# GlassyWing/yolo_deepsort

Measured on AMD Instinct MI355X. Metric: end-to-end frames/sec (detect+ReID+assoc), 608x608, higher is better.
Workload: dtype f16x3

## Files before the change

include/ydsort.h:

```cpp
#ifndef YDSORT_H
#define YDSORT_H

#include <stddef.h>
#include <stdint.h>

#ifdef __cplusplus
extern "C" {
#endif

typedef struct yds_net yds_net;
typedef struct yds_reid yds_reid;
typedef struct yds_trk yds_trk;
typedef struct yds_pipe yds_pipe;
typedef struct yds_zones yds_zones;
typedef struct yds_heatmap yds_heatmap;
typedef struct yds_act yds_act;
typedef struct yds_ident yds_ident;
typedef struct yds_comm yds_comm;

int yds_init(int device_id);
int yds_current_device(void);
int yds_device_pci_bus_id(char *buf, int len);
const char *yds_last_error(void);
int yds_device_count(void);
// ... 13 lines not shown
int yds_darknet_set_batch_max(yds_net *, int batch_max);
int yds_darknet_batch_max(const yds_net *);
int yds_darknet_set_half(yds_net *, int on);
int yds_darknet_layer_format(const yds_net *, int layer);
int yds_darknet_num_boxes(const yds_net *);
int yds_darknet_num_attrs(const yds_net *);
int yds_darknet_num_layers(const yds_net *);
int yds_darknet_layer_shape(const yds_net *, int layer, int *c, int *h, int *w);
int64_t yds_darknet_conv_flops(const yds_net *);
int yds_darknet_forward_f32(yds_net *, const float *nchw_host, int batch, float *out_host);
int yds_darknet_forward_u8(yds_net *, const uint8_t *rgb_hwc_host, int h, int w, int batch,
                           float *out_host_or_null);
int yds_darknet_forward_u8_dev(yds_net *, const uint8_t *rgb_hwc_dev, int h, int w, int batch);
int yds_darknet_forward_u8_mixed_dev(yds_net *, const uint8_t *rgb_hwc_dev, const uint64_t *frame_off, const int32_t *frame_hw ,
                                     size_t frames_bytes, int batch);
const uint8_t *yds_darknet_last_frames_dev(yds_net *, int *h, int *w, int *batch);
int yds_darknet_layer_output(yds_net *, int layer, int batch, float *nchw_host);
int yds_darknet_get_input(yds_net *, int batch, float *nchw_host);

int yds_nms(yds_net *, int image, float conf_thres, double iou_thres, int frame_h, int frame_w,
            float *out6_host, int cap, int *n_out);
int yds_nms_pred(const float *pred_host, int n_boxes, int attrs, float conf_thres, double iou_thres,
                 float *out6_host, int cap, int *n_out);

int yds_detect_tiled(yds_net *, const uint8_t *rgb_hwc_host, int h, int w, const int32_t *tiles_xyhw, int n_tiles,
                     float conf_thres, double iou_thres, float *out6_host, int cap, int *n_out);
int yds_nms_merge_pred(const float *pred_host, int n_boxes, int attrs, float conf_thres, double iou_thres,
                       float *out6_host, int cap, int *n_out);
int yds_nms_merge_pred_batched(const float *pred_host, int n_frames, int n_boxes, int attrs, float conf_thres, double iou_thres,
                               float *out6_host, int cap, int *n_out);
int yds_nms_ragged_pred(const float *pred_host, size_t total_rows, int attrs, int n_frames, const uint64_t *row0, const int32_t *n_rows,
                        const int32_t *corner_merge, const float *scale, float conf_thres, double iou_thres, float *out6_host, int cap,
                        int *n_out);

yds_reid *yds_reid_create(int max_crops);
void yds_reid_destroy(yds_reid *);
int yds_reid_load_tensor(yds_reid *, const char *name, const float *data_host, const int64_t *shape, int ndim);
int yds_reid_finalize(yds_reid *);
int64_t yds_reid_flops_per_crop(void);
int yds_reid_embed(yds_reid *, const uint8_t *frame_rgb_host, int h, int w, const float *tlwh_host,
                   int D, float *out_host);
int yds_reid_embed_dev(yds_reid *, const uint8_t *frame_rgb_dev, int h, int w, const float *tlwh_host,
                       int D, float *out_host_or_null);
const float *yds_reid_features_dev(yds_reid *);
int yds_reid_preprocess(yds_reid *, const uint8_t *frame_rgb_host, int h, int w, const float *tlwh_host,
                        int D, float *nchw_host);
// ... 240 lines not shown
```

yolo_deepsort_amd/_lib.py:

```python

from __future__ import annotations

import ctypes as C
import os

import numpy as np

HERE = os.path.dirname(os.path.abspath(__file__))
_TAG = os.environ.get("YDS_BUILD_TAG", "")
LIB_PATH = os.path.join(HERE, "libydsort" + ("_" + _TAG if _TAG else "") + ".so")


class YdsError(RuntimeError):
    pass


_P = C.c_void_p
_I = C.c_int
_F = C.c_float
_D = C.c_double
_SZ = C.c_size_t
_I64 = C.c_int64

SIGNATURES = {
# ... 170 lines not shown
    "yds_pipeline_set_zones": (_I, [_P, _P]),
    "yds_pipeline_last_zone_events": (_I, [_P, _P, _P, _I, _P]),
    "yds_heatmap_create": (_P, [_I, _I]),
    "yds_heatmap_destroy": (None, [_P]),
    "yds_heatmap_set_stream": (_I, [_P, _I, _I, _I, _I, _I]),
    "yds_heatmap_reset": (_I, [_P, _I]),
    "yds_heatmap_update": (_I, [_P, _P, _P, _P, _P, _I, _P]),
    "yds_heatmap_get_layers": (_I, [_P, _I, _P, _SZ]),
    "yds_heatmap_get_max": (_I, [_P, _I, _I, _P]),
    "yds_heatmap_get_tracks": (_I, [_P, _I, _P, _P, _P, _P, _P, _I, _P]),
    "yds_heatmap_render": (_I, [_P, _P, _I, _P, _P, _I, _I, _I, _I, _I64, _I, _P]),
    "yds_heatmap_set_timing": (_I, [_P, _I]),
    "yds_heatmap_last_us": (_I, [_P, _I, _P]),
    "yds_pipeline_set_heatmap": (_I, [_P, _P]),
    "yds_overlay_tracks_masked": (_I, [_P, _I, _P, _I, _I, _I, _P, _P, _P, _I, _P, _P, _I, _I, _I, _P, _P, _I, _I, C.c_uint32, _P, _P]),
    "yds_overlay_tracks_bgr_masked": (_I, [_P, _I, _P, _I, _I, _I, _P, _P, _P, _I, _P, _P, _I, _I, _I, _P, _P, _I, _I, C.c_uint32, _P]),
    "yds_anonymize_frames": (_I, [_P, _I, _P, _I, _I, _I, _P, _P, _I, _I, C.c_uint32]),
    "yds_pipeline_last_detections": (_I, [_P, _P, _I, _P]),
    "yds_overlay_tracks_mixed": (_I, [_P, _SZ, _I, _P, _P, _P, _I, _P, _P, _P, _I, _P, _P, _I, _I, _P, _P, _I, _I, C.c_uint32, _P, _SZ, _P]),
    "yds_overlay_tracks_bgr_mixed": (_I, [_P, _SZ, _I, _P, _P, _P, _I, _P, _P, _P, _I, _P, _P, _I, _I, _P, _P, _I, _I, C.c_uint32, _P]),
    "yds_anonymize_frames_mixed": (_I, [_P, _SZ, _I, _P, _P, _P, _I, _P, _P, _I, _I, C.c_uint32]),
    "yds_overlay_set_timing": (_I, [_I]),
    "yds_overlay_last_us": (_I, [_P]),
}

_lib = None
MISSING = []


def load():
    global _lib
    if _lib is not None:
        return _lib
    if not os.path.exists(LIB_PATH):
        raise YdsError(f"{LIB_PATH} not found: build it with `python -m yolo_deepsort_amd.build` "
                       "(the product has no CPU fallback)")
    lib = C.CDLL(LIB_PATH)
    for name, (res, args) in SIGNATURES.items():
        try:
            fn = getattr(lib, name)
        except AttributeError:
            MISSING.append(name)
            continue
        fn.restype = res
        fn.argtypes = args
    _lib = lib
# ... 128 lines not shown
```

yolo_deepsort_amd/csrc/common.h:

```cpp
#pragma once
#include <hip/hip_runtime.h>
#include <stdint.h>
#include <stdio.h>
#include <string>
#include <vector>
#include <stdexcept>

#include "slot_plan.h"

namespace yds {

void set_error(const std::string &msg);
struct Error : std::runtime_error {
    explicit Error(const std::string &m) : std::runtime_error(m) {}
};
[[noreturn]] void fail(const char *fmt, ...);
int bound_device();
void bind_thread();
hipStream_t make_stream(bool latency_role);

#define YDS_HIP(expr)                                                                          \
    do {                                                                                       \
        hipError_t _e = (expr);                                                                \
        if (_e != hipSuccess)                                                                  \
// ... 86 lines not shown
int launch_conv(const ConvArgs &a, hipStream_t s, int variant = -1);
constexpr int kVariantMask = 0xff, kTileGnShift = 8;
bool conv_presplit_input(const ConvArgs &a);
bool launch_conv_maxpool3s2(const ConvArgs &a, hipStream_t s);
int conv_autotune(const ConvArgs &a, hipStream_t s, float *best_us);
std::vector<int> conv_candidates(const ConvArgs &a);
enum ConvMath { MATH_F32 = 0, MATH_F16X3 = 1 };
int conv_math();
void set_conv_math(int m);
void pack_weights_f16x3(const float *w, int cout, int kpad, std::vector<uint16_t> &out);
const char *conv_variant_name(int v);
double conv_flops(const ConvArgs &a);
double conv_bytes_io(const View &v);
double conv_bytes(const ConvArgs &a);

void launch_maxpool(const View &x, const View &y, int k, int stride, int pad, bool zero_pad_br, hipStream_t s);
void launch_upsample(const View &x, const View &y, int stride, hipStream_t s);
void launch_copy(const View &x, const View &y, hipStream_t s);
void launch_add(const View &a, const View &b, const View &y, hipStream_t s);
void launch_nchw_to_nhwc(const float *src_nchw, const View &y, int c_src, hipStream_t s);
void launch_nhwc_to_nchw(const View &x, float *dst_nchw, hipStream_t s);
void nhwc_to_host(const View &x, float *dst_nchw_host, hipStream_t s);
void launch_pack_h16(const float *src_f32, const View &y, hipStream_t s);
void launch_yolo_decode(const View &head, float *out, int total_boxes, int box_off, int num_classes,
                        const float *anchors_wh , int A, int img_h, int img_w, hipStream_t s);
void launch_inject(const View &head, int image, const float *rows_dev, int n, int head_index, int num_classes,
                   float logit, hipStream_t s);
void launch_inject_batch(const View &head, int batch, const float *table_dev, const int *offsets_dev, int max_rows, int head_index,
                         int num_classes, float logit, hipStream_t s);
void launch_resize_u8(const uint8_t *frames, int n, int h, int w, const View &y, hipStream_t s, bool bgr = false);
std::vector<FrameGeom> checked_layout(const uint64_t *frame_off, const int32_t *frame_hw, int n, size_t frames_bytes);
void launch_slot_resize(const uint8_t *frames, const SlotRec *slots, int n, const View &y, hipStream_t s, bool bgr);
void launch_slot_boxes(const float *pred, int n_boxes, int attrs, const SlotRec *slots, int n, float *dst, hipStream_t s);
struct ReidFront {
    const uint8_t *frames = nullptr;
    const FrameGeom *geom = nullptr;
    const int *boxes = nullptr;
    int h = 0, w = 0, bgr = 0;
};
void launch_crop_resize(const ReidFront &f, int D, const View &y, hipStream_t s);
void launch_reid_stem(const ReidFront &f, int D, const float *w, int kpad, const float *bias, const View &pooled, hipStream_t s);
constexpr int kReidStemUnitsPerCrop = 4;
int reid_stem_grid();
void launch_avgpool_l2norm(const View &x, float *out, hipStream_t s);

}
```

yolo_deepsort_amd/csrc/darknet.cpp:

```cpp
#include "engine.h"
#include "h16.h"
#include "conv_common.h"

#include <math.h>
#include <stdlib.h>
#include <string.h>
#include <map>
#include <sstream>

namespace yds {

std::vector<CfgBlock> parse_cfg(const std::string &text) {
    std::vector<CfgBlock> blocks;
    std::istringstream in(text);
    std::string line;
    auto strip = [](std::string s) {
        size_t a = s.find_first_not_of(" \t\r\n"), b = s.find_last_not_of(" \t\r\n");
        return a == std::string::npos ? std::string() : s.substr(a, b - a + 1);
    };
    while (std::getline(in, line)) {
        if (line.empty() || line[0] == '#') continue;
        line = strip(line);
        if (line.empty()) fail("cfg: whitespace-only line (the reference parser rejects it too)");
        if (line[0] == '[') {
// ... 584 lines not shown
        switch (st.kind) {
        case Step::CONV: case Step::CONV_MERGED: case Step::CONV_STEM2: case Step::CONV_BLOCK1:
            enqueue_conv(st, first, batch, stream);
            break;
        case Step::MAXPOOL: launch_maxpool(v(st.src), v(i), st.ksize, st.stride, st.pad, st.zero_br, stream); break;
        case Step::UPSAMPLE: launch_upsample(v(l.src), v(i), l.stride, stream); break;
        case Step::COPY: {
            View d = v(i);
            d.p += fmt_slots(d.fmt, st.arg);
            launch_copy(v(st.src), d, stream);
            break;
        }
        case Step::ADD: launch_add(v(l.refs[0]), v(l.refs[1]), v(i), stream); break;
        case Step::YOLO: {
            const View head = v(l.src);
            const int hidx = st.arg;
            if (inject_active && inject_set >= 0) {
                launch_inject_batch(head, batch, inject_table.p, inject_offsets_dev.p + (size_t)inject_set * batch_max + first, inject_max_rows, hidx,
                                    l.classes, inject_logit, stream);
            } else {
                for (int b = 0; b < batch && inject_active; ++b)
                    launch_inject(head, b, inject_rows[first + b].p, inject_n[first + b], hidx, l.classes, inject_logit, stream);
            }
            launch_yolo_decode(head, out.p + (size_t)first * total_boxes * attrs, total_boxes, l.box_off, l.classes, l.anchors.data(), (int)l.anchors.size() / 2, img_h, img_w, stream);
            break;
        }
        }
    }
}

void Darknet::forward_f32_host(const float *nchw, int batch, float *out_host) {
    size_t n = (size_t)batch * in_channels * img_h * img_w;
    YDS_HIP(hipMemcpyAsync(stage_f32.p, nchw, n * sizeof(float), hipMemcpyHostToDevice, stream));
    launch_nchw_to_nhwc(stage_f32.p, input_view(batch), in_channels, stream);
    run_graph(batch);
    if (out_host) YDS_HIP(hipMemcpyAsync(out_host, out.p, (size_t)batch * total_boxes * attrs * sizeof(float), hipMemcpyDeviceToHost, stream));
    YDS_HIP(hipStreamSynchronize(stream));
}

void Darknet::forward_u8_dev(const uint8_t *frames_dev, int h, int w, int batch) {
    if (in_channels != 3) fail("forward_u8: network expects %d channels", in_channels);
    check_pass(batch);
    launch_resize_u8(frames_dev, batch, h, w, input_view(batch), stream);
    run_graph(batch);
}

void Darknet::forward_u8_frames_dev(const uint8_t *frames_dev, const std::vector<FrameGeom> &geom) {
// ... 283 lines not shown
```

yolo_deepsort_amd/csrc/engine.h:

```cpp
#pragma once
#include "common.h"
#include "conv_weights.h"

#include <map>
#include <memory>
#include <string>
#include <utility>
#include <vector>

namespace yds {

struct CfgBlock {
    std::string type;
    std::map<std::string, std::string> kv;
};
std::vector<CfgBlock> parse_cfg(const std::string &text);

enum LayerType { L_CONV, L_MAXPOOL, L_UPSAMPLE, L_ROUTE, L_SHORTCUT, L_YOLO };

struct Layer {
    LayerType type = L_CONV;
    int c = 0, h = 0, w = 0;
    int root = -1, coff = 0;
    int src = -1;
// ... 70 lines not shown
    bool half_mode = false;
    void set_half(bool on);
    void plan_half_formats();
    int owner_of(int layer, int &off) const;
    int total_boxes = 0, attrs = 0;
    std::vector<Layer> layers;
    std::vector<Storage> storage;
    std::vector<int> yolo_layers;
    DevBuf<float> input, out, stage_f32;
    DevBuf<uint8_t> stage_u8;
    DevBuf<SlotRec> slot_tab;
    int stage_h = 0, stage_w = 0, stage_n = 0;
    DevBuf<float> tiled_pred;
    hipStream_t stream = nullptr;
    std::vector<DevBuf<float>> inject_rows;
    std::vector<int> inject_n;
    bool inject_active = false;
    DevBuf<float> inject_table;
    std::vector<int> inject_offsets;
    DevBuf<int> inject_offsets_dev;
    int inject_max_rows = 0;
    int inject_set = -1;
    float inject_logit = 6.f;
    struct ConvTimeRec { hipEvent_t e0 = nullptr, e1 = nullptr; int variant = 0; double flops = 0, bytes = 0, attain_us = 0; };
    bool time_convs = false;
    std::vector<ConvTimeRec> conv_pending;
    std::vector<hipEvent_t> ev_pool;
    hipEvent_t timing_event();
    void resolve_conv_timing();
    double conv_us[kConvVariants] = {}, conv_flops_acc[kConvVariants] = {}, conv_bytes_acc[kConvVariants] = {}, conv_attain_us[kConvVariants] = {};
    int64_t conv_launches[kConvVariants] = {};

private:
    void allocate_buffers();
    void check_pass(int batch) const;
    void run_graph(int batch);
    void run_lane(int first, int batch, hipStream_t st, int l0 = 0, int l1 = -1);
    void enqueue_conv(const Step &st, int first, int batch, hipStream_t s);
    const LaunchPlan &plan(int batch);
    LaunchPlan plan_;
    int plan_epoch = 0;
    bool stem_fusable = false;
    int block1_at = -1;
    std::vector<hipStream_t> lane_streams;
    std::vector<hipEvent_t> lane_done;
    hipEvent_t lane_fork = nullptr;
};

struct NmsUniform { int32_t n_boxes, corner, merge; float sx, sy; };
class NmsWorkspace {
public:
    explicit NmsWorkspace(int max_candidates = 16384, int frames = 1);
    ~NmsWorkspace();
    NmsWorkspace(const NmsWorkspace &) = delete;
    void launch(const float *pred_dev, const NmsUniform &u, int n_frames, int attrs, float conf_thres, double iou_thres, int cap, hipStream_t s);
    void launch(const float *pred_dev, const NmsFrame *fr, int n_frames, int max_rows, size_t total_rows, int attrs, float conf_thres,
                double iou_thres, int cap, hipStream_t s);
    int collect(int frame, float *out6_host, int cap);
    void resize(int max_candidates, int n_frames);
    int needed(int n_frames) const;
    static constexpr int kMaxCandidates = 1 << 18;
    int run(const float *pred_dev, int n_boxes, int attrs, float conf_thres, double iou_thres, float sx, float sy,
            float *out6_host, int cap, hipStream_t s);
    int run_merge(const float *pred_dev, int n_boxes, int attrs, float conf_thres, double iou_thres, float *out6_host, int cap, hipStream_t s);
    int max_cand, frames;
    DevBuf<float> cand;
    DevBuf<float> sorted;
    DevBuf<int> counts;
    DevBuf<int> box_count;
    DevBuf<unsigned long long> mask;
    DevBuf<float> kept;
    int *h_counts = nullptr;
    float *h_kept = nullptr;
};

class ReidNet {
public:
    explicit ReidNet(int max_crops);
// ... 117 lines not shown
```

yolo_deepsort_amd/csrc/layers.hip:

```cpp
#include "common.h"

#include <algorithm>
#include "h16.h"
#include "resize_dev.h"

namespace yds {

static inline int grid_for(size_t work, int block = 256) {
    size_t g = (work + block - 1) / block;
    if (g > 8192) g = 8192;
    if (g < 1) g = 1;
    return (int)g;
}

__global__ void maxpool_kernel(const float *x, float *y, int N, int H, int W, int C, int ldx, int Ho, int Wo, int ldy,
                               int k, int stride, int pad, int zero_br, int fmt_in, int fmt_out) {
    fp16_saturate_on();
    const int C4 = C >> 2;
    const size_t total = (size_t)N * Ho * Wo * C4;
    for (size_t idx = blockIdx.x * (size_t)blockDim.x + threadIdx.x; idx < total; idx += (size_t)gridDim.x * blockDim.x) {
        int c4 = idx % C4;
        size_t pix = idx / C4;
        int ox = pix % Wo;
        size_t t = pix / Wo;
        int oy = t % Ho;
// ... 172 lines not shown
    const int wave0 = __builtin_amdgcn_readfirstlane((int)((blockIdx.x * blockDim.x + threadIdx.x) >> 6));
    const int nwaves = (int)((gridDim.x * blockDim.x) >> 6);
    for (int cell = wave0; cell < HW; cell += nwaves) {
        const int gy = cell / W, gx = cell - gy * W;
        const float *src = head + ((size_t)(n * H + gy) * W + gx) * ld;
        float *dst = out + ((size_t)n * total_boxes + box_off + cell) * attrs;
        for (int i = lane; i < per_cell; i += 64) {
            int a = 0;
#pragma unroll
            for (int k = 1; k < 8; ++k) a += (k < A && i >= k * attrs) ? 1 : 0;
            const int t = i - a * attrs;
            const float v = src[i];
            float r;
            if (t == 0) r = __fmul_rn(__fadd_rn(1.f / (1.f + expf(-v)), (float)gx), yp.s0);
            else if (t == 1) r = __fmul_rn(__fadd_rn(1.f / (1.f + expf(-v)), (float)gy), yp.s1);
            else if (t == 2) r = __fmul_rn(__fmul_rn(expf(v), yp.aw[a]), yp.s0);
            else if (t == 3) r = __fmul_rn(__fmul_rn(expf(v), yp.ah[a]), yp.s1);
            else r = 1.f / (1.f + expf(-v));
            dst[(size_t)a * HW * attrs + t] = r;
        }
    }
}

void launch_yolo_decode(const View &head, float *out, int total_boxes, int box_off, int num_classes, const float *anchors_wh,
                        int A, int img_h, int img_w, hipStream_t s) {
    if (A > 8) fail("yolo: at most 8 anchors per head");
    YoloParams yp;
    yp.s0 = (float)((double)img_h / head.h);
    yp.s1 = (float)((double)img_w / head.w);
    for (int a = 0; a < A; ++a) {
        yp.aw[a] = anchors_wh[2 * a] / yp.s0;
        yp.ah[a] = anchors_wh[2 * a + 1] / yp.s1;
    }
    int attrs = num_classes + 5;
    if (head.c != A * attrs) fail("yolo: head has %d channels, expected %d", head.c, A * attrs);
    const size_t per_img = (size_t)A * head.h * head.w * attrs;
    if (per_img >= (1ull << 31)) fail("yolo: head too large for 32-bit indexing");
    const unsigned cells = (unsigned)head.h * head.w;
    hipLaunchKernelGGL(yolo_decode_kernel, dim3(std::min((cells + 3) / 4, 2048u), head.n), dim3(256), 0, s, head.p, out, head.n, head.h, head.w,
                       head.ld, A, attrs, total_boxes, box_off, yp);
    YDS_HIP(hipGetLastError());
}

__global__ void inject_clear_kernel(float *head, int image, int H, int W, int ld, int A, int attrs, float logit) {
    int total = H * W * A;
    for (int idx = blockIdx.x * blockDim.x + threadIdx.x; idx < total; idx += gridDim.x * blockDim.x) {
        int a = idx % A, cell = idx / A;
        head[((size_t)image * H * W + cell) * ld + a * attrs + 4] = -logit;
    }
}
__device__ __forceinline__ bool inject_row_superseded(const float *rows, int r, int n) {
    const float *row = rows + (size_t)r * 9;
    for (int j = r + 1; j < n; ++j) {
        const float *o = rows + (size_t)j * 9;
        if (o[0] == row[0] && o[1] == row[1] && o[2] == row[2] && o[3] == row[3]) return true;
    }
    return false;
}
__global__ void inject_rows_kernel(float *head, int image, int H, int W, int ld, int attrs, const float *rows, int n, int head_index,
                                   float logit) {
    int r = blockIdx.x;
    if (r >= n) return;
    const float *row = rows + r * 9;
    if ((int)row[0] != head_index) return;
// ... 193 lines not shown
```

yolo_deepsort_amd/csrc/nms.hip:

```cpp
#include "engine.h"

#include <string.h>

#include <vector>

namespace yds {

constexpr int MAX_DET = 300;

__device__ __forceinline__ NmsFrame frame_at(const NmsUniform &u, int f) {
    return NmsFrame{(uint64_t)f * u.n_boxes, u.n_boxes, u.corner, u.merge, u.sx, u.sy, 0};
}
__device__ __forceinline__ NmsFrame frame_at(const NmsFrame *fr, int f) { return fr[f]; }

__device__ __forceinline__ void nms_count_body(const float *pred, int n_boxes, int attrs, float thr, int *box_count) {
    int i = blockIdx.x * blockDim.x + threadIdx.x;
    if (i >= n_boxes) return;
    const float *p = pred + (size_t)i * attrs;
    int cnt = 0;
    float obj = p[4];
    if (obj > thr) {
        for (int j = 5; j < attrs; ++j) cnt += __fmul_rn(p[j], obj) > thr;
    }
    box_count[i] = cnt;
// ... 14 lines not shown
        int v = i < n_boxes ? box_count[i] : 0;
        int incl = v;
        for (int o = 1; o < 64; o <<= 1) {
            int t = __shfl_up(incl, o, 64);
            if (lane >= o) incl += t;
        }
        if (lane == 63) wave_sum[wave] = incl;
        __syncthreads();
        int woff = 0;
        for (int w = 0; w < wave; ++w) woff += wave_sum[w];
        int c = carry;
        if (i < n_boxes) box_count[i] = c + woff + incl - v;
        __syncthreads();
        if (tid == (int)blockDim.x - 1) carry = c + woff + incl;
        __syncthreads();
    }
    if (tid == 0) { counts[0] = carry; counts[1] = 0; }
}
template <class Frames> __global__ void nms_scan_kernel(int *box_count, Frames frames, int *counts_all) {
    const NmsFrame f = frame_at(frames, blockIdx.y);
    nms_scan_body(box_count + f.row0, f.n_rows, counts_all + blockIdx.y * 4);
}

__device__ __forceinline__ void nms_emit_body(const float *pred, int n_boxes, int attrs, float thr, const int *box_off, int max_cand, float *cand,
                                              int corner) {
    int i = blockIdx.x * blockDim.x + threadIdx.x;
    if (i >= n_boxes) return;
    const float *p = pred + (size_t)i * attrs;
    float obj = p[4];
    if (!(obj > thr)) return;
    int slot = box_off[i];
    float x1 = p[0], y1 = p[1], x2 = p[2], y2 = p[3];
    if (!corner) {
        float hw = __fdiv_rn(p[2], 2.f), hh = __fdiv_rn(p[3], 2.f);
        x1 = __fsub_rn(p[0], hw); y1 = __fsub_rn(p[1], hh); x2 = __fadd_rn(p[0], hw); y2 = __fadd_rn(p[1], hh);
    }
    for (int j = 5; j < attrs; ++j) {
        float sc = __fmul_rn(p[j], obj);
        if (sc > thr) {
            if (slot < max_cand) {
                float *r = cand + (size_t)slot * 6;
                r[0] = x1; r[1] = y1; r[2] = x2; r[3] = y2; r[4] = sc; r[5] = (float)(j - 5);
            }
            ++slot;
        }
    }
}
template <class Frames>
__global__ void nms_emit_kernel(const float *pred, Frames frames, int attrs, float thr, const int *box_off, int max_cand, float *cand_all) {
    const NmsFrame f = frame_at(frames, blockIdx.y);
    nms_emit_body(pred + (size_t)f.row0 * attrs, f.n_rows, attrs, thr, box_off + f.row0, max_cand, cand_all + (size_t)blockIdx.y * max_cand * 6, f.corner);
}

__global__ void nms_rank_kernel(const float *cand_all, const int *counts_all, int max_cand, float *sorted_all) {
    const float *cand = cand_all + (size_t)blockIdx.y * max_cand * 6;
    float *sorted = sorted_all + (size_t)blockIdx.y * max_cand * 6;
    const int *counts = counts_all + blockIdx.y * 4;
    __shared__ float tile[256];
    const int n = min(counts[0], max_cand);
    for (int base = blockIdx.x * blockDim.x; base < n; base += gridDim.x * blockDim.x) {
        int i = base + threadIdx.x;
        float si = i < n ? cand[(size_t)i * 6 + 4] : 0.f;
        int rank = 0;
        for (int t0 = 0; t0 < n; t0 += 256) {
            int j = t0 + threadIdx.x;
            tile[threadIdx.x] = j < n ? cand[(size_t)j * 6 + 4] : -INFINITY;
            __syncthreads();
            int lim = min(256, n - t0);
            for (int k = 0; k < lim; ++k) {
                float sj = tile[k];
                rank += (sj > si) || (sj == si && (t0 + k) < i);
            }
            __syncthreads();
        }
// ... 148 lines not shown
        mean[threadIdx.x] = __fdiv_rn((float)acc, wsum);
    }
    __syncthreads();
    for (int i = threadIdx.x; i < k * 4; i += blockDim.x) kept[(size_t)(i >> 2) * 6 + (i & 3)] = mean[i & 3];
}
template <class Frames>
__global__ __launch_bounds__(256) void nms_merge_kernel(const float *cand_all, const float *sorted_all, const int *counts_all, int max_cand,
                                                        float iou_thres, Frames frames, float *kept_all) {
    if (!frame_at(frames, blockIdx.x).merge) return;
    nms_merge_body(cand_all, sorted_all, counts_all, max_cand, iou_thres, kept_all);
}

__global__ __launch_bounds__(256) void nms_publish_kernel(const int *counts, const float *kept, int *h_counts, float *h_kept, int cap) {
    const int f = blockIdx.x;
    if (threadIdx.x < 4) h_counts[f * 4 + threadIdx.x] = counts[f * 4 + threadIdx.x];
    const int n = min(counts[f * 4 + 1], cap) * 6;
    const float *src = kept + (size_t)f * MAX_DET * 6;
    float *dst = h_kept + (size_t)f * MAX_DET * 6;
    for (int i = threadIdx.x; i < n; i += 256) dst[i] = src[i];
}

template <class Frames>
static void launch_stages(NmsWorkspace &w, const float *pred_dev, Frames frames, int n_frames, int max_rows, size_t total_rows, bool merge, int attrs,
                          float conf_thres, double iou_thres, int cap, hipStream_t s) {
    if (attrs < 6) fail("nms: predictions need at least one class");
    if (n_frames < 1 || max_rows < 1) fail("nms: %d frames of at most %d rows", n_frames, max_rows);
    if (n_frames > w.frames) w.resize(w.max_cand, n_frames);
    w.box_count.ensure(total_rows);
    const int nb = (max_rows + 255) / 256, max_cand = w.max_cand, words_ld = max_cand / 64;
    hipLaunchKernelGGL(nms_count_kernel<Frames>, dim3(nb, n_frames), dim3(256), 0, s, pred_dev, frames, attrs, conf_thres, w.box_count.p);
    hipLaunchKernelGGL(nms_scan_kernel<Frames>, dim3(1, n_frames), dim3(1024), 0, s, w.box_count.p, frames, w.counts.p);
    hipLaunchKernelGGL(nms_emit_kernel<Frames>, dim3(nb, n_frames), dim3(256), 0, s, pred_dev, frames, attrs, conf_thres, w.box_count.p, max_cand,
                       w.cand.p);
    hipLaunchKernelGGL(nms_rank_kernel, dim3(16, n_frames), dim3(256), 0, s, w.cand.p, w.counts.p, max_cand, w.sorted.p);
    hipLaunchKernelGGL(nms_mask_kernel, dim3(64, n_frames), dim3(256), 0, s, w.sorted.p, w.counts.p, max_cand, iou_thres, w.mask.p, words_ld);
    hipLaunchKernelGGL(nms_sweep_kernel<Frames>, dim3(1, n_frames), dim3(256), words_ld * sizeof(unsigned long long), s, w.sorted.p, w.mask.p, words_ld,
                       w.counts.p, max_cand, frames, w.kept.p, cap);
    if (merge)
        hipLaunchKernelGGL(nms_merge_kernel<Frames>, dim3(n_frames), dim3(256), 0, s, w.cand.p, w.sorted.p, w.counts.p, max_cand, (float)iou_thres, frames,
                           w.kept.p);
    hipLaunchKernelGGL(nms_publish_kernel, dim3(n_frames), dim3(256), 0, s, w.counts.p, w.kept.p, w.h_counts, w.h_kept, std::min(cap, (int)MAX_DET));
    YDS_HIP(hipGetLastError());
}

void NmsWorkspace::launch(const float *pred_dev, const NmsUniform &u, int n_frames, int attrs, float conf_thres, double iou_thres, int cap,
                          hipStream_t s) {
    launch_stages(*this, pred_dev, u, n_frames, u.n_boxes, (size_t)std::max(frames, n_frames) * u.n_boxes, u.merge != 0, attrs, conf_thres,
                  iou_thres, cap, s);
}

void NmsWorkspace::launch(const float *pred_dev, const NmsFrame *fr, int n_frames, int max_rows, size_t total_rows, int attrs, float conf_thres,
                          double iou_thres, int cap, hipStream_t s) {
    launch_stages(*this, pred_dev, fr, n_frames, max_rows, total_rows, true, attrs, conf_thres, iou_thres, cap, s);
}

template <class Launch> static void launch_grown(NmsWorkspace &w, int n_frames, hipStream_t s, Launch launch) {
    launch();
    YDS_HIP(hipStreamSynchronize(s));
    if (w.needed(n_frames) <= w.max_cand) return;
    w.resize(w.needed(n_frames), w.frames);
    launch();
    YDS_HIP(hipStreamSynchronize(s));
}

int NmsWorkspace::collect(int frame, float *out6_host, int cap) {
    const int *c = h_counts + frame * 4;
    if (c[0] > max_cand) fail("nms: %d candidates exceed the workspace capacity %d (caller must resize and relaunch)", c[0], max_cand);
    int n = c[1] < cap ? c[1] : cap;
    if (n > 0) memcpy(out6_host, h_kept + (size_t)frame * MAX_DET * 6, (size_t)n * 6 * sizeof(float));
    return n;
}

int NmsWorkspace::run(const float *pred_dev, int n_boxes, int attrs, float conf_thres, double iou_thres, float sx, float sy,
                      float *out6_host, int cap, hipStream_t s) {
    launch_grown(*this, 1, s, [&] { launch(pred_dev, NmsUniform{n_boxes, 0, 0, sx, sy}, 1, attrs, conf_thres, iou_thres, cap, s); });
    return collect(0, out6_host, cap);
}

int NmsWorkspace::run_merge(const float *pred_dev, int n_boxes, int attrs, float conf_thres, double iou_thres, float *out6_host, int cap,
                            hipStream_t s) {
    launch_grown(*this, 1, s, [&] { launch(pred_dev, NmsUniform{n_boxes, 1, 1, 1.f, 1.f}, 1, attrs, conf_thres, iou_thres, MAX_DET, s); });
    return collect(0, out6_host, cap);
}

}


namespace {
yds::NmsWorkspace &workspace() {
    static thread_local std::unique_ptr<yds::NmsWorkspace> ws;
    if (!ws) ws.reset(new yds::NmsWorkspace());
    return *ws;
}
yds::NmsWorkspace &frames_workspace(int n_frames) {
    static thread_local std::unique_ptr<yds::NmsWorkspace> ws;
    if (!ws) ws.reset(new yds::NmsWorkspace(4096, n_frames));
    return *ws;
}
}

extern "C" {

int yds_nms(yds_net *n, int image, float conf_thres, double iou_thres, int frame_h, int frame_w, float *out6_host, int cap, int *n_out) {
    YDS_API_BEGIN
// ... 23 lines not shown
    *n_out = workspace().run_merge(pred.p, n_boxes, attrs, conf_thres, iou_thres, out6_host, cap, nullptr);
    YDS_API_END
}

int yds_nms_ragged_pred(const float *pred_host, size_t total_rows, int attrs, int n_frames, const uint64_t *row0, const int32_t *n_rows,
                        const int32_t *corner_merge, const float *scale, float conf_thres, double iou_thres, float *out6_host, int cap, int *n_out) {
    YDS_API_BEGIN
    if (n_frames < 1) yds::fail("nms: %d frames", n_frames);
    std::vector<yds::NmsFrame> fr(n_frames);
    int max_rows = 0;
    for (int f = 0; f < n_frames; ++f) {
        if (n_rows[f] < 1 || row0[f] + (uint64_t)n_rows[f] > total_rows)
            yds::fail("nms: frame %d holds rows [%llu, +%d) of %zu", f, (unsigned long long)row0[f], n_rows[f], total_rows);
        fr[f] = yds::NmsFrame{row0[f], n_rows[f], corner_merge[f * 2] != 0, corner_merge[f * 2 + 1] != 0, scale[f * 2], scale[f * 2 + 1], 0};
        max_rows = std::max(max_rows, n_rows[f]);
    }
    yds::NmsWorkspace &ws = frames_workspace(n_frames);
    yds::DevBuf<float> pred;
    yds::DevBuf<yds::NmsFrame> fr_dev;
    pred.upload(pred_host, total_rows * attrs);
    fr_dev.upload(fr.data(), fr.size());
    YDS_HIP(hipStreamSynchronize(nullptr));
    yds::launch_grown(ws, n_frames, nullptr,
                      [&] { ws.launch(pred.p, fr_dev.p, n_frames, max_rows, total_rows, attrs, conf_thres, iou_thres, yds::MAX_DET, nullptr); });
    for (int f = 0; f < n_frames; ++f) n_out[f] = ws.collect(f, out6_host + (size_t)f * cap * 6, cap);
    YDS_API_END
}

int yds_nms_merge_pred_batched(const float *pred_host, int n_frames, int n_boxes, int attrs, float conf_thres, double iou_thres, float *out6_host,
                               int cap, int *n_out) {
    YDS_API_BEGIN
    if (n_frames < 1 || n_boxes < 1) yds::fail("nms: %d frames of %d boxes", n_frames, n_boxes);
    yds::NmsWorkspace &ws = frames_workspace(n_frames);
    yds::DevBuf<float> pred;
    pred.upload(pred_host, (size_t)n_frames * n_boxes * attrs);
    YDS_HIP(hipStreamSynchronize(nullptr));
    yds::launch_grown(ws, n_frames, nullptr, [&] {
        ws.launch(pred.p, yds::NmsUniform{n_boxes, 1, 1, 1.f, 1.f}, n_frames, attrs, conf_thres, iou_thres, yds::MAX_DET, nullptr);
    });
    for (int f = 0; f < n_frames; ++f) n_out[f] = ws.collect(f, out6_host + (size_t)f * cap * 6, cap);
    YDS_API_END
}

int yds_nms_pred(const float *pred_host, int n_boxes, int attrs, float conf_thres, double iou_thres, float *out6_host, int cap, int *n_out) {
    YDS_API_BEGIN
    yds::DevBuf<float> pred;
    pred.upload(pred_host, (size_t)n_boxes * attrs);
    YDS_HIP(hipStreamSynchronize(nullptr));
    *n_out = workspace().run(pred.p, n_boxes, attrs, conf_thres, iou_thres, 1.f, 1.f, out6_host, cap, nullptr);
    YDS_API_END
}

}
```

yolo_deepsort_amd/csrc/pipeline.cpp:

```cpp
#include "engine.h"

#include <limits.h>
#include <stdlib.h>
#include <string.h>

#include <algorithm>
#include <chrono>
#include <utility>

namespace yds {

struct DetSlot {
    std::unique_ptr<NmsWorkspace> nms;
    hipEvent_t e0, e1, e2, e_nms;
    hipEvent_t e_r0, e_r1;
    bool reid_in_pass = false;
    DetSlot() { for (hipEvent_t *e : {&e0, &e1, &e2, &e_nms, &e_r0, &e_r1}) YDS_HIP(hipEventCreate(e)); }
    ~DetSlot() {
        for (hipEvent_t e : {e0, e1, e2, e_nms, e_r0, e_r1}) (void)hipEventDestroy(e);
        if (plan_tab) (void)hipHostFree(plan_tab);
    }
    void *plan_tab = nullptr;
    size_t plan_bytes = 0, plan_slots_n = 0;
    const SlotRec *plan_slots() const { return static_cast<const SlotRec *>(plan_tab); }
// ... 156 lines not shown
        if (p.done == Pass::HEAD) launch_detector_tail(p);
    }
    void launch_detector_head(Pass &p, bool split) {
        DetSlot &s = det[p.slot];
        s.reid_in_pass = false;
        stager.wait_uploaded(p.frames, net->stream);
        YDS_HIP(hipEventRecord(s.e0, net->stream));
        p.done = Pass::HEAD;
        p.split = false;
        if (!p.plan.empty()) s.write_plan(p.plan);
        if (p.plan.windowed) {
            YDS_HIP(hipEventRecord(s.e1, net->stream));
            return;
        }
        if (p.plan.direct()) launch_slot_resize(p.frames, s.plan_slots(), p.batch, net->input_view(p.batch), net->stream, frames_bgr);
        else launch_resize_u8(p.frames, p.batch, p.geo.h, p.geo.w, net->input_view(p.batch), net->stream, frames_bgr);
        YDS_HIP(hipEventRecord(s.e1, net->stream));
        stager.mark_read(p.frames, net->stream, FrameStager::DET);
        p.split = split && net->forward_resized_part(p.batch, 0);
    }
    void launch_detector_tail(Pass &p) {
        DetSlot &s = det[p.slot];
        const size_t per_slot = (size_t)net->total_boxes * net->attrs, n_slots = p.plan.slots.size();
        if (p.plan.windowed) {
            if (win_pred.n < n_slots * per_slot) {
                YDS_HIP(hipStreamSynchronize(net->stream));
                win_pred.alloc(n_slots * per_slot);
            }
            pred_rows = n_slots * net->total_boxes;
            net->forward_slots(p.frames, s.plan_slots(), (int)n_slots, win_pred.p, frames_bgr);
            stager.mark_read(p.frames, net->stream, FrameStager::DET);
        } else if (p.split) {
            (void)net->forward_resized_part(p.batch, 1);
        } else {
            net->forward_resized(p.batch);
        }
        YDS_HIP(hipEventRecord(s.e2, net->stream));
        if (p.plan.empty()) {
            const float sx = box_scale(p.geo.w, net->img_w), sy = box_scale(p.geo.h, net->img_h);
            s.nms->launch(net->out.p, NmsUniform{net->total_boxes, 0, 0, sx, sy}, p.batch, net->attrs, conf, nms_thres, 300, net->stream);
        } else {
            s.nms->launch(p.plan.windowed ? win_pred.p : net->out.p, s.plan_frames(), p.batch, p.plan.max_rows, n_slots * net->total_boxes,
                          net->attrs, conf, nms_thres, 300, net->stream);
        }
        YDS_HIP(hipEventRecord(s.e_nms, net->stream));
        p.done = Pass::WHOLE;
    }

    void set_windows(int ww, int wh, double overlap) {
        if (pending.frames || ahead.reid_in_flight) fail("pipeline: set_windows while a look-ahead pass is in flight (consume it with a step first)");
        if (ww > 0 && wh <= 0) fail("pipeline: window %d x %d", ww, wh);
        if (ww > 0 && !(overlap >= 0)) fail("pipeline: window overlap %g", overlap);
        if (ww > 0 && any_stream_windows()) fail("pipeline: set_windows while a stream holds a window setting of its own (set_stream_windows): one or the other");
        win_w = ww > 0 ? ww : 0; win_h = ww > 0 ? wh : 0; win_overlap = overlap;
    }
    bool any_stream_windows() const {
        for (const WindowSetting &sw : stream_win)
            if (sw.w > 0) return true;
        return false;
    }
    void set_stream_windows(int stream, int ww, int wh, double overlap) {
        if (!multi) fail("pipeline: created by yds_pipeline_create: it has no streams (window mode: yds_pipeline_set_windows)");
        if (stream < 0 || stream >= (int)trks.size()) fail("pipeline: stream %d outside [0,%zu)", stream, trks.size());
// ... 509 lines not shown
```

Before: 1685.

## Fuse NMS candidate counting into a wave-per-cell YOLO decode kernel

Adds a YOLO decode kernel that gives each 64-lane wave a run of cells, prefetches the next cell's head values, and computes per-anchor class counts above the confidence threshold with ballots. The counts go straight into the NMS workspace's box_count buffer, so the pipeline can skip the separate NMS count kernel, which re-read the whole prediction tensor. The emit stage now checks for empty slots using the scan offsets rather than relying only on objectness. In exchange it adds a second decode path, extra coupling state between the network and the pipeline, and test entry points; the fused counting is only used for unplanned, non-split passes.

Result: no change. 1696 (median of 6 runs) (+0.6%).

```diff
diff --git a/include/ydsort.h b/include/ydsort.h
--- a/include/ydsort.h
+++ b/include/ydsort.h
@@ -59,6 +59,13 @@
             float *out6_host, int cap, int *n_out);
 int yds_nms_pred(const float *pred_host, int n_boxes, int attrs, float conf_thres, double iou_thres,
                  float *out6_host, int cap, int *n_out);
+
+int yds_decode_force_generic(int on);
+int yds_yolo_decode(const float *head_host, int n, int h, int w, int ld, int A, int num_classes, const float *anchors_wh, int img_h,
+                    int img_w, int total_boxes, int box_off, float count_thr, float *out_host, int32_t *box_count_host, int *counted);
+int yds_nms_count_pred(const float *pred_host, int n_frames, int n_boxes, int attrs, float conf_thres, int32_t *box_count_host);
+int yds_decode_nms(const float *head_host, int n, int h, int w, int ld, int A, int num_classes, const float *anchors_wh, int img_h,
+                   int img_w, float conf_thres, double iou_thres, int max_cand, float *out6_host, int *n_out, int *info);
 
 int yds_detect_tiled(yds_net *, const uint8_t *rgb_hwc_host, int h, int w, const int32_t *tiles_xyhw, int n_tiles,
                      float conf_thres, double iou_thres, float *out6_host, int cap, int *n_out);
diff --git a/yolo_deepsort_amd/_lib.py b/yolo_deepsort_amd/_lib.py
--- a/yolo_deepsort_amd/_lib.py
+++ b/yolo_deepsort_amd/_lib.py
@@ -216,6 +216,10 @@
     "yds_anonymize_frames_mixed": (_I, [_P, _SZ, _I, _P, _P, _P, _I, _P, _P, _I, _I, C.c_uint32]),
     "yds_overlay_set_timing": (_I, [_I]),
     "yds_overlay_last_us": (_I, [_P]),
+    "yds_decode_force_generic": (_I, [_I]),
+    "yds_yolo_decode": (_I, [_P, _I, _I, _I, _I, _I, _I, _P, _I, _I, _I, _I, _F, _P, _P, _P]),
+    "yds_nms_count_pred": (_I, [_P, _I, _I, _I, _F, _P]),
+    "yds_decode_nms": (_I, [_P, _I, _I, _I, _I, _I, _I, _P, _I, _I, _F, _D, _I, _P, _P, _P]),
 }
 
 _lib = None
diff --git a/yolo_deepsort_amd/csrc/common.h b/yolo_deepsort_amd/csrc/common.h
--- a/yolo_deepsort_amd/csrc/common.h
+++ b/yolo_deepsort_amd/csrc/common.h
@@ -132,8 +132,11 @@
 void launch_nhwc_to_nchw(const View &x, float *dst_nchw, hipStream_t s);
 void nhwc_to_host(const View &x, float *dst_nchw_host, hipStream_t s);
 void launch_pack_h16(const float *src_f32, const View &y, hipStream_t s);
-void launch_yolo_decode(const View &head, float *out, int total_boxes, int box_off, int num_classes,
-                        const float *anchors_wh , int A, int img_h, int img_w, hipStream_t s);
+bool launch_yolo_decode(const View &head, float *out, int total_boxes, int box_off, int num_classes,
+                        const float *anchors_wh , int A, int img_h, int img_w, hipStream_t s, float count_thr = 0.f,
+                        int *box_count = nullptr);
+bool decode_generic();
+void set_decode_generic(bool on);
 void launch_inject(const View &head, int image, const float *rows_dev, int n, int head_index, int num_classes,
                    float logit, hipStream_t s);
 void launch_inject_batch(const View &head, int batch, const float *table_dev, const int *offsets_dev, int max_rows, int head_index,
diff --git a/yolo_deepsort_amd/csrc/darknet.cpp b/yolo_deepsort_amd/csrc/darknet.cpp
--- a/yolo_deepsort_amd/csrc/darknet.cpp
+++ b/yolo_deepsort_amd/csrc/darknet.cpp
@@ -630,7 +630,10 @@
                 for (int b = 0; b < batch && inject_active; ++b)
                     launch_inject(head, b, inject_rows[first + b].p, inject_n[first + b], hidx, l.classes, inject_logit, stream);
             }
-            launch_yolo_decode(head, out.p + (size_t)first * total_boxes * attrs, total_boxes, l.box_off, l.classes, l.anchors.data(), (int)l.anchors.size() / 2, img_h, img_w, stream);
+            const bool wrote = launch_yolo_decode(head, out.p + (size_t)first * total_boxes * attrs, total_boxes, l.box_off, l.classes, l.anchors.data(),
+                                                  (int)l.anchors.size() / 2, img_h, img_w, stream, count_thr,
+                                                  count_dst ? count_dst + (size_t)first * total_boxes : nullptr);
+            counted = counted && wrote;
             break;
         }
         }
diff --git a/yolo_deepsort_amd/csrc/engine.h b/yolo_deepsort_amd/csrc/engine.h
--- a/yolo_deepsort_amd/csrc/engine.h
+++ b/yolo_deepsort_amd/csrc/engine.h
@@ -116,6 +116,9 @@
     int inject_max_rows = 0;
     int inject_set = -1;
     float inject_logit = 6.f;
+    int *count_dst = nullptr;
+    float count_thr = 0.f;
+    bool counted = false;
     struct ConvTimeRec { hipEvent_t e0 = nullptr, e1 = nullptr; int variant = 0; double flops = 0, bytes = 0, attain_us = 0; };
     bool time_convs = false;
     std::vector<ConvTimeRec> conv_pending;
@@ -147,7 +150,9 @@
     explicit NmsWorkspace(int max_candidates = 16384, int frames = 1);
     ~NmsWorkspace();
     NmsWorkspace(const NmsWorkspace &) = delete;
-    void launch(const float *pred_dev, const NmsUniform &u, int n_frames, int attrs, float conf_thres, double iou_thres, int cap, hipStream_t s);
+    void launch(const float *pred_dev, const NmsUniform &u, int n_frames, int attrs, float conf_thres, double iou_thres, int cap, hipStream_t s,
+                bool counted = false);
+    int *count_rows(int n_frames, int n_boxes);
     void launch(const float *pred_dev, const NmsFrame *fr, int n_frames, int max_rows, size_t total_rows, int attrs, float conf_thres,
                 double iou_thres, int cap, hipStream_t s);
     int collect(int frame, float *out6_host, int cap);
diff --git a/yolo_deepsort_amd/csrc/layers.hip b/yolo_deepsort_amd/csrc/layers.hip
--- a/yolo_deepsort_amd/csrc/layers.hip
+++ b/yolo_deepsort_amd/csrc/layers.hip
@@ -1,6 +1,7 @@
 #include "common.h"
 
 #include <algorithm>
+#include <atomic>
 #include "h16.h"
 #include "resize_dev.h"
 
@@ -219,24 +220,119 @@
     }
 }
 
-void launch_yolo_decode(const View &head, float *out, int total_boxes, int box_off, int num_classes, const float *anchors_wh,
-                        int A, int img_h, int img_w, hipStream_t s) {
+constexpr int DEC_TRIPS = 4, DEC_CELLS = 8;
+__global__ __launch_bounds__(256) void yolo_decode_fast_kernel(const float *head, float *out, int H, int W, int ld, int A, int attrs, int total_boxes,
+                                                              int box_off, YoloParams yp, float thr, int *box_count) {
+    const int HW = H * W, n = blockIdx.y, per_cell = A * attrs;
+    const int lane = threadIdx.x & 63;
+    int tk[DEC_TRIPS], an[DEC_TRIPS], doff[DEC_TRIPS];
+    float anc[DEC_TRIPS], sc[DEC_TRIPS];
+#pragma unroll
+    for (int k = 0; k < DEC_TRIPS; ++k) {
+        const int i = lane + 64 * k;
+        int a = 0;
+#pragma unroll
+        for (int j = 1; j < 8; ++j) a += (j < A && i >= j * attrs) ? 1 : 0;
+        const int t = i - a * attrs;
+        float aw = 0.f, ah = 0.f;
+#pragma unroll
+        for (int j = 0; j < 8; ++j) { aw = a == j ? yp.aw[j] : aw; ah = a == j ? yp.ah[j] : ah; }
+        tk[k] = i < per_cell ? (t < 5 ? t : 5) : 6;
+        an[k] = a;
+        doff[k] = a * HW * attrs + t;
+        anc[k] = t == 2 ? aw : ah;
+        sc[k] = (t == 0 || t == 2) ? yp.s0 : yp.s1;
+    }
+    const int wave0 = __builtin_amdgcn_readfirstlane((int)((blockIdx.x * blockDim.x + threadIdx.x) >> 6));
+    const int nwaves = (int)((gridDim.x * blockDim.x) >> 6);
+    for (int c0 = wave0 * DEC_CELLS; c0 < HW; c0 += nwaves * DEC_CELLS) {
+        const int c1 = min(HW, c0 + DEC_CELLS);
+        const float *src = head + ((size_t)n * HW + c0) * ld;
+        float *dst = out + ((size_t)n * total_boxes + box_off + c0) * attrs;
+        int *cnt_dst = box_count ? box_count + (size_t)n * total_boxes + box_off + c0 : nullptr;
+        float v[DEC_TRIPS], nv[DEC_TRIPS];
+#pragma unroll
+        for (int k = 0; k < DEC_TRIPS; ++k) v[k] = tk[k] < 6 ? src[lane + 64 * k] : 0.f;
+        for (int cell = c0; cell < c1; ++cell) {
+            src += ld;
+#pragma unroll
+            for (int k = 0; k < DEC_TRIPS; ++k) nv[k] = (cell + 1 < c1 && tk[k] < 6) ? src[lane + 64 * k] : 0.f;
+            const int gy = cell / W, gx = cell - gy * W;
+            const float fx = (float)gx, fy = (float)gy;
+            float r[DEC_TRIPS];
+#pragma unroll
+            for (int k = 0; k < DEC_TRIPS; ++k) {
+                const bool wh = tk[k] == 2 || tk[k] == 3;
+                const float e = expf(wh ? v[k] : -v[k]);
+                const float sig = 1.f / (1.f + e);
+                const float x = wh ? __fmul_rn(e, anc[k]) : __fadd_rn(sig, tk[k] == 0 ? fx : fy);
+                r[k] = tk[k] >= 4 ? sig : __fmul_rn(x, sc[k]);
+                if (tk[k] < 6) dst[doff[k]] = r[k];
+            }
+            if (cnt_dst) {
+                int mine = 0;
+                for (int a = 0; a < A; ++a) {
+                    const int oi = a * attrs + 4, ot = oi >> 6;
+                    const float ov = ot == 0 ? r[0] : ot == 1 ? r[1] : ot == 2 ? r[2] : r[3];
+                    const float obj = __int_as_float(__builtin_amdgcn_readlane(__float_as_int(ov), __builtin_amdgcn_readfirstlane(oi & 63)));
+                    int cnt = 0;
+                    if (obj > thr) {
+#pragma unroll
+                        for (int k = 0; k < DEC_TRIPS; ++k)
+                            cnt += __popcll(__ballot(tk[k] == 5 && an[k] == a && __fmul_rn(r[k], obj) > thr));
+                    }
+                    mine = lane == a ? cnt : mine;
+                }
+                if (lane < A) cnt_dst[lane * HW] = mine;
+                ++cnt_dst;
+            }
+            dst += attrs;
+#pragma unroll
+            for (int k = 0; k < DEC_TRIPS; ++k) v[k] = nv[k];
+        }
+    }
+}
+
+static std::atomic<int> g_decode_generic{-1};
+bool decode_generic() {
+    int v = g_decode_generic.load();
+    if (v < 0) {
+        const char *e = getenv("YDS_DECODE_GENERIC");
+        v = (e && atoi(e) != 0) ? 1 : 0;
+        g_decode_generic.store(v);
+    }
+    return v != 0;
+}
+void set_decode_generic(bool on) { g_decode_generic.store(on ? 1 : 0); }
+
+bool launch_yolo_decode(const View &head, float *out, int total_boxes, int box_off, int num_classes, const float *anchors_wh,
+                        int A, int img_h, int img_w, hipStream_t s, float count_thr, int *box_count) {
     if (A > 8) fail("yolo: at most 8 anchors per head");
     YoloParams yp;
     yp.s0 = (float)((double)img_h / head.h);
     yp.s1 = (float)((double)img_w / head.w);
+    for (int a = 0; a < 8; ++a) yp.aw[a] = yp.ah[a] = 0.f;
     for (int a = 0; a < A; ++a) {
         yp.aw[a] = anchors_wh[2 * a] / yp.s0;
         yp.ah[a] = anchors_wh[2 * a + 1] / yp.s1;
     }
     int attrs = num_classes + 5;
     if (head.c != A * attrs) fail("yolo: head has %d channels, expected %d", head.c, A * attrs);
+    if (head.ld < head.c) fail("yolo: head stride %d below its %d channels", head.ld, head.c);
     const size_t per_img = (size_t)A * head.h * head.w * attrs;
     if (per_img >= (1ull << 31)) fail("yolo: head too large for 32-bit indexing");
     const unsigned cells = (unsigned)head.h * head.w;
-    hipLaunchKernelGGL(yolo_decode_kernel, dim3(std::min((cells + 3) / 4, 2048u), head.n), dim3(256), 0, s, head.p, out, head.n, head.h, head.w,
-                       head.ld, A, attrs, total_boxes, box_off, yp);
-    YDS_HIP(hipGetLastError());
+    const bool fast = A * attrs <= 64 * DEC_TRIPS && !decode_generic();
+    if (fast) {
+        const unsigned chunks = (cells + DEC_CELLS - 1) / DEC_CELLS;
+        hipLaunchKernelGGL(yolo_decode_fast_kernel, dim3(std::min((chunks + 3) / 4, 2048u), head.n), dim3(256), 0, s, head.p, out, head.h, head.w,
+                           head.ld, A, attrs, total_boxes, box_off, yp, count_thr, box_count);
+    } else {
+        hipLaunchKernelGGL(yolo_decode_kernel, dim3(std::min((cells + 3) / 4, 2048u), head.n), dim3(256), 0, s, head.p, out, head.n, head.h, head.w,
+                           head.ld, A, attrs, total_boxes, box_off, yp);
+    }
+    YDS_HIP(hipGetLastError());
+    return fast && box_count != nullptr;
 }
 
 __global__ void inject_clear_kernel(float *head, int image, int H, int W, int ld, int A, int attrs, float logit) {
diff --git a/yolo_deepsort_amd/csrc/nms.hip b/yolo_deepsort_amd/csrc/nms.hip
--- a/yolo_deepsort_amd/csrc/nms.hip
+++ b/yolo_deepsort_amd/csrc/nms.hip
@@ -60,14 +60,15 @@
     nms_scan_body(box_count + f.row0, f.n_rows, counts_all + blockIdx.y * 4);
 }
 
-__device__ __forceinline__ void nms_emit_body(const float *pred, int n_boxes, int attrs, float thr, const int *box_off, int max_cand, float *cand,
-                                              int corner) {
+__device__ __forceinline__ void nms_emit_body(const float *pred, int n_boxes, int attrs, float thr, const int *box_off, int total, int max_cand,
+                                              float *cand, int corner) {
     int i = blockIdx.x * blockDim.x + threadIdx.x;
     if (i >= n_boxes) return;
+    int slot = box_off[i];
+    if ((i + 1 < n_boxes ? box_off[i + 1] : total) == slot) return;
     const float *p = pred + (size_t)i * attrs;
     float obj = p[4];
     if (!(obj > thr)) return;
-    int slot = box_off[i];
     float x1 = p[0], y1 = p[1], x2 = p[2], y2 = p[3];
     if (!corner) {
         float hw = __fdiv_rn(p[2], 2.f), hh = __fdiv_rn(p[3], 2.f);
@@ -85,9 +86,11 @@
     }
 }
 template <class Frames>
-__global__ void nms_emit_kernel(const float *pred, Frames frames, int attrs, float thr, const int *box_off, int max_cand, float *cand_all) {
+__global__ void nms_emit_kernel(const float *pred, Frames frames, int attrs, float thr, const int *box_off, const int *counts_all, int max_cand,
+                                float *cand_all) {
     const NmsFrame f = frame_at(frames, blockIdx.y);
-    nms_emit_body(pred + (size_t)f.row0 * attrs, f.n_rows, attrs, thr, box_off + f.row0, max_cand, cand_all + (size_t)blockIdx.y * max_cand * 6, f.corner);
+    nms_emit_body(pred + (size_t)f.row0 * attrs, f.n_rows, attrs, thr, box_off + f.row0, counts_all[blockIdx.y * 4], max_cand,
+                  cand_all + (size_t)blockIdx.y * max_cand * 6, f.corner);
 }
 
 __global__ void nms_rank_kernel(const float *cand_all, const int *counts_all, int max_cand, float *sorted_all) {
@@ -282,15 +285,17 @@
 
 template <class Frames>
 static void launch_stages(NmsWorkspace &w, const float *pred_dev, Frames frames, int n_frames, int max_rows, size_t total_rows, bool merge, int attrs,
-                          float conf_thres, double iou_thres, int cap, hipStream_t s) {
+                          float conf_thres, double iou_thres, int cap, hipStream_t s, bool counted = false) {
     if (attrs < 6) fail("nms: predictions need at least one class");
     if (n_frames < 1 || max_rows < 1) fail("nms: %d frames of at most %d rows", n_frames, max_rows);
     if (n_frames > w.frames) w.resize(w.max_cand, n_frames);
+    if (counted && w.box_count.n < total_rows) fail("nms: the counts of %zu rows were announced, the buffer holds %zu", total_rows, w.box_count.n);
     w.box_count.ensure(total_rows);
     const int nb = (max_rows + 255) / 256, max_cand = w.max_cand, words_ld = max_cand / 64;
-    hipLaunchKernelGGL(nms_count_kernel<Frames>, dim3(nb, n_frames), dim3(256), 0, s, pred_dev, frames, attrs, conf_thres, w.box_count.p);
+    if (!counted)
+        hipLaunchKernelGGL(nms_count_kernel<Frames>, dim3(nb, n_frames), dim3(256), 0, s, pred_dev, frames, attrs, conf_thres, w.box_count.p);
     hipLaunchKernelGGL(nms_scan_kernel<Frames>, dim3(1, n_frames), dim3(1024), 0, s, w.box_count.p, frames, w.counts.p);
-    hipLaunchKernelGGL(nms_emit_kernel<Frames>, dim3(nb, n_frames), dim3(256), 0, s, pred_dev, frames, attrs, conf_thres, w.box_count.p, max_cand,
+    hipLaunchKernelGGL(nms_emit_kernel<Frames>, dim3(nb, n_frames), dim3(256), 0, s, pred_dev, frames, attrs, conf_thres, w.box_count.p, w.counts.p, max_cand,
                        w.cand.p);
     hipLaunchKernelGGL(nms_rank_kernel, dim3(16, n_frames), dim3(256), 0, s, w.cand.p, w.counts.p, max_cand, w.sorted.p);
     hipLaunchKernelGGL(nms_mask_kernel, dim3(64, n_frames), dim3(256), 0, s, w.sorted.p, w.counts.p, max_cand, iou_thres, w.mask.p, words_ld);
@@ -304,9 +309,14 @@
 }
 
 void NmsWorkspace::launch(const float *pred_dev, const NmsUniform &u, int n_frames, int attrs, float conf_thres, double iou_thres, int cap,
-                          hipStream_t s) {
+                          hipStream_t s, bool counted) {
     launch_stages(*this, pred_dev, u, n_frames, u.n_boxes, (size_t)std::max(frames, n_frames) * u.n_boxes, u.merge != 0, attrs, conf_thres,
-                  iou_thres, cap, s);
+                  iou_thres, cap, s, counted);
+}
+
+int *NmsWorkspace::count_rows(int n_frames, int n_boxes) {
+    box_count.ensure((size_t)std::max(frames, n_frames) * n_boxes);
+    return box_count.p;
 }
 
 void NmsWorkspace::launch(const float *pred_dev, const NmsFrame *fr, int n_frames, int max_rows, size_t total_rows, int attrs, float conf_thres,
@@ -315,11 +325,11 @@
 }
 
 template <class Launch> static void launch_grown(NmsWorkspace &w, int n_frames, hipStream_t s, Launch launch) {
-    launch();
+    launch(false);
     YDS_HIP(hipStreamSynchronize(s));
     if (w.needed(n_frames) <= w.max_cand) return;
     w.resize(w.needed(n_frames), w.frames);
-    launch();
+    launch(true);
     YDS_HIP(hipStreamSynchronize(s));
 }
 
@@ -333,13 +343,13 @@
 
 int NmsWorkspace::run(const float *pred_dev, int n_boxes, int attrs, float conf_thres, double iou_thres, float sx, float sy,
                       float *out6_host, int cap, hipStream_t s) {
-    launch_grown(*this, 1, s, [&] { launch(pred_dev, NmsUniform{n_boxes, 0, 0, sx, sy}, 1, attrs, conf_thres, iou_thres, cap, s); });
+    launch_grown(*this, 1, s, [&](bool) { launch(pred_dev, NmsUniform{n_boxes, 0, 0, sx, sy}, 1, attrs, conf_thres, iou_thres, cap, s); });
     return collect(0, out6_host, cap);
 }
 
 int NmsWorkspace::run_merge(const float *pred_dev, int n_boxes, int attrs, float conf_thres, double iou_thres, float *out6_host, int cap,
                             hipStream_t s) {
-    launch_grown(*this, 1, s, [&] { launch(pred_dev, NmsUniform{n_boxes, 1, 1, 1.f, 1.f}, 1, attrs, conf_thres, iou_thres, MAX_DET, s); });
+    launch_grown(*this, 1, s, [&](bool) { launch(pred_dev, NmsUniform{n_boxes, 1, 1, 1.f, 1.f}, 1, attrs, conf_thres, iou_thres, MAX_DET, s); });
     return collect(0, out6_host, cap);
 }
 
@@ -409,7 +419,7 @@
     fr_dev.upload(fr.data(), fr.size());
     YDS_HIP(hipStreamSynchronize(nullptr));
     yds::launch_grown(ws, n_frames, nullptr,
-                      [&] { ws.launch(pred.p, fr_dev.p, n_frames, max_rows, total_rows, attrs, conf_thres, iou_thres, yds::MAX_DET, nullptr); });
+                      [&](bool) { ws.launch(pred.p, fr_dev.p, n_frames, max_rows, total_rows, attrs, conf_thres, iou_thres, yds::MAX_DET, nullptr); });
     for (int f = 0; f < n_frames; ++f) n_out[f] = ws.collect(f, out6_host + (size_t)f * cap * 6, cap);
     YDS_API_END
 }
@@ -422,10 +432,77 @@
     yds::DevBuf<float> pred;
     pred.upload(pred_host, (size_t)n_frames * n_boxes * attrs);
     YDS_HIP(hipStreamSynchronize(nullptr));
-    yds::launch_grown(ws, n_frames, nullptr, [&] {
+    yds::launch_grown(ws, n_frames, nullptr, [&](bool) {
         ws.launch(pred.p, yds::NmsUniform{n_boxes, 1, 1, 1.f, 1.f}, n_frames, attrs, conf_thres, iou_thres, yds::MAX_DET, nullptr);
     });
     for (int f = 0; f < n_frames; ++f) n_out[f] = ws.collect(f, out6_host + (size_t)f * cap * 6, cap);
+    YDS_API_END
+}
+
+int yds_decode_force_generic(int on) {
+    YDS_API_BEGIN
+    yds::set_decode_generic(on != 0);
+    YDS_API_END
+}
+
+int yds_yolo_decode(const float *head_host, int n, int h, int w, int ld, int A, int num_classes, const float *anchors_wh, int img_h, int img_w,
+                    int total_boxes, int box_off, float count_thr, float *out_host, int32_t *box_count_host, int *counted) {
+    YDS_API_BEGIN
+    if (n < 1 || h < 1 || w < 1 || A < 1 || num_classes < 1) yds::fail("yolo: a head of %d x %d x %d, %d anchors, %d classes", n, h, w, A, num_classes);
+    const int attrs = num_classes + 5;
+    if (ld < A * attrs) yds::fail("yolo: head stride %d below its %d channels", ld, A * attrs);
+    if (box_off < 0 || (size_t)box_off + (size_t)A * h * w > (size_t)total_boxes) yds::fail("yolo: boxes [%d, +%d) outside %d", box_off, A * h * w, total_boxes);
+    const size_t rows = (size_t)n * total_boxes;
+    yds::DevBuf<float> head, out(rows * attrs);
+    yds::DevBuf<int> cnt(rows);
+    head.upload(head_host, (size_t)n * h * w * ld);
+    YDS_HIP(hipMemsetAsync(out.p, 0, rows * attrs * sizeof(float), nullptr));
+    YDS_HIP(hipMemsetAsync(cnt.p, 0xff, rows * sizeof(int), nullptr));
+    yds::View v;
+    v.p = head.p; v.n = n; v.h = h; v.w = w; v.c = A * attrs; v.ld = ld;
+    *counted = yds::launch_yolo_decode(v, out.p, total_boxes, box_off, num_classes, anchors_wh, A, img_h, img_w, nullptr, count_thr,
+                                       box_count_host ? cnt.p : nullptr) ? 1 : 0;
+    YDS_HIP(hipMemcpyAsync(out_host, out.p, rows * attrs * sizeof(float), hipMemcpyDeviceToHost, nullptr));
+    if (box_count_host) YDS_HIP(hipMemcpyAsync(box_count_host, cnt.p, rows * sizeof(int), hipMemcpyDeviceToHost, nullptr));
+    YDS_HIP(hipStreamSynchronize(nullptr));
+    YDS_API_END
+}
+
+int yds_nms_count_pred(const float *pred_host, int n_frames, int n_boxes, int attrs, float conf_thres, int32_t *box_count_host) {
+    YDS_API_BEGIN
+    if (n_frames < 1 || n_boxes < 1 || attrs < 6) yds::fail("nms: %d frames of %d boxes, %d values each", n_frames, n_boxes, attrs);
+    const size_t rows = (size_t)n_frames * n_boxes;
+    yds::DevBuf<float> pred;
+    yds::DevBuf<int> cnt(rows);
+    pred.upload(pred_host, rows * attrs);
+    hipLaunchKernelGGL(yds::nms_count_kernel<yds::NmsUniform>, dim3((n_boxes + 255) / 256, n_frames), dim3(256), 0, nullptr, pred.p,
+                       yds::NmsUniform{n_boxes, 0, 0, 1.f, 1.f}, attrs, conf_thres, cnt.p);
+    YDS_HIP(hipGetLastError());
+    YDS_HIP(hipMemcpyAsync(box_count_host, cnt.p, rows * sizeof(int), hipMemcpyDeviceToHost, nullptr));
+    YDS_HIP(hipStreamSynchronize(nullptr));
+    YDS_API_END
+}
+
+int yds_decode_nms(const float *head_host, int n, int h, int w, int ld, int A, int num_classes, const float *anchors_wh, int img_h, int img_w,
+                   float conf_thres, double iou_thres, int max_cand, float *out6_host, int *n_out, int *info) {
+    YDS_API_BEGIN
+    if (n < 1 || h < 1 || w < 1 || A < 1 || num_classes < 1) yds::fail("yolo: a head of %d x %d x %d, %d anchors, %d classes", n, h, w, A, num_classes);
+    const int attrs = num_classes + 5, n_boxes = A * h * w;
+    if (ld < A * attrs) yds::fail("yolo: head stride %d below its %d channels", ld, A * attrs);
+    yds::NmsWorkspace ws(max_cand, n);
+    yds::DevBuf<float> head, pred((size_t)n * n_boxes * attrs);
+    head.upload(head_host, (size_t)n * h * w * ld);
+    yds::View v;
+    v.p = head.p; v.n = n; v.h = h; v.w = w; v.c = A * attrs; v.ld = ld;
+    const bool counted = yds::launch_yolo_decode(v, pred.p, n_boxes, 0, num_classes, anchors_wh, A, img_h, img_w, nullptr, conf_thres,
+                                                 ws.count_rows(n, n_boxes));
+    int runs = 0;
+    yds::launch_grown(ws, n, nullptr, [&](bool rerun) {
+        ++runs;
+        ws.launch(pred.p, yds::NmsUniform{n_boxes, 0, 0, 1.f, 1.f}, n, attrs, conf_thres, iou_thres, yds::MAX_DET, nullptr, counted && !rerun);
+    });
+    for (int f = 0; f < n; ++f) n_out[f] = ws.collect(f, out6_host + (size_t)f * yds::MAX_DET * 6, yds::MAX_DET);
+    info[0] = counted ? 1 : 0; info[1] = runs; info[2] = ws.max_cand;
     YDS_API_END
 }
 
diff --git a/yolo_deepsort_amd/csrc/pipeline.cpp b/yolo_deepsort_amd/csrc/pipeline.cpp
--- a/yolo_deepsort_amd/csrc/pipeline.cpp
+++ b/yolo_deepsort_amd/csrc/pipeline.cpp
@@ -202,6 +202,16 @@
     void launch_detector_tail(Pass &p) {
         DetSlot &s = det[p.slot];
         const size_t per_slot = (size_t)net->total_boxes * net->attrs, n_slots = p.plan.slots.size();
+        const bool count_in_decode = p.plan.empty() && !(p.split && !net->yolo_layers.empty() && net->yolo_layers.front() < net->head_layers());
+        struct CountsOff {
+            Darknet *net;
+            ~CountsOff() { net->count_dst = nullptr; net->counted = false; }
+        } counts_off{net};
+        if (count_in_decode) {
+            net->count_dst = s.nms->count_rows(p.batch, net->total_boxes);
+            net->count_thr = conf;
+            net->counted = true;
+        }
         if (p.plan.windowed) {
             if (win_pred.n < n_slots * per_slot) {
                 YDS_HIP(hipStreamSynchronize(net->stream));
@@ -216,9 +226,10 @@
             net->forward_resized(p.batch);
         }
         YDS_HIP(hipEventRecord(s.e2, net->stream));
+        const bool counted = count_in_decode && net->counted;
         if (p.plan.empty()) {
             const float sx = box_scale(p.geo.w, net->img_w), sy = box_scale(p.geo.h, net->img_h);
-            s.nms->launch(net->out.p, NmsUniform{net->total_boxes, 0, 0, sx, sy}, p.batch, net->attrs, conf, nms_thres, 300, net->stream);
+            s.nms->launch(net->out.p, NmsUniform{net->total_boxes, 0, 0, sx, sy}, p.batch, net->attrs, conf, nms_thres, 300, net->stream, counted);
         } else {
             s.nms->launch(p.plan.windowed ? win_pred.p : net->out.p, s.plan_frames(), p.batch, p.plan.max_rows, n_slots * net->total_boxes,
                           net->attrs, conf, nms_thres, 300, net->stream);
```
